# KentaYoshii/Raymarcher

Hardware: AMD Instinct MI355X
Metric: Mpixels/s at 3840x2160 Mandelbulb, 256 march steps (higher is better)
Workload: dtype f32

## Files before the change

raymarcher_amd/csrc/rm_device.hip.h:

```cpp
#pragma once
#include "../../include/raymarcher_amd.h"
#include <type_traits>

#include "rm_math.hip.h"
#include "rm_internal.h"

namespace rm {

struct V3 { float x, y, z; };
struct V4 { float x, y, z, w; };

RM_DEV V3 v3(float x, float y, float z) { return V3{x, y, z}; }
RM_DEV V4 v4(float x, float y, float z, float w) { return V4{x, y, z, w}; }
RM_DEV V3 add(V3 a, V3 b) { return v3(a.x + b.x, a.y + b.y, a.z + b.z); }
RM_DEV V3 sub(V3 a, V3 b) { return v3(a.x - b.x, a.y - b.y, a.z - b.z); }
RM_DEV V3 mul(V3 a, V3 b) { return v3(a.x * b.x, a.y * b.y, a.z * b.z); }
RM_DEV V3 scale(V3 a, float s) { return v3(a.x * s, a.y * s, a.z * s); }
RM_DEV V3 neg(V3 a) { return v3(-a.x, -a.y, -a.z); }
RM_DEV V3 madd(V3 a, float s, V3 b) { return v3(fma(a.x, s, b.x), fma(a.y, s, b.y), fma(a.z, s, b.z)); }
RM_DEV float dot2(float ax, float ay, float bx, float by) { return fma(ay, by, ax * bx); }
RM_DEV float dot(V3 a, V3 b) { return fma(a.z, b.z, fma(a.y, b.y, a.x * b.x)); }
RM_DEV float len2(float x, float y) { return sqrt_(dot2(x, y, x, y)); }
RM_DEV float len(V3 a) { return sqrt_(dot(a, a)); }
RM_DEV V3 normalize(V3 a) { float inv = rcp_(len(a)); return scale(a, inv); }
// ... 472 lines not shown
  const float lipLen = SKIP ? (sb->cullLip * len(rd)) * 1.0001f : 0.0f;
  float ub = ub0;
  float second = -__builtin_inff();
  for (int i = 0; i < steps; i++) {
    const V3 p = madd(rd, depth, ro);
    bool one = false;
    int nearU = 0;
    if (SKIP) {
      nearU = __builtin_amdgcn_readfirstlane(c.idx);
      one = sb->cullOneOk && __ballot(!(c.idx == nearU && nearU >= 0 && second > ub)) == 0ull;
    }
    if (SKIP && one) c = sdSceneOne<COUNT>(sb, nearU, p, cnt);
    else c = sdSceneImpl<BULB, COUNT, !SHADOW, SKIP, SKIP>(sb, p, cnt, ub, second);
    if (fabs_(c.d) < kSurfaceDist || depth > end) break;
    if (SHADOW) {
      if (soft) pen = min_(pen, divr_(8.0f * c.d, depth));
      depth = depth + fabs_(c.d);
    } else {
      depth = fma(c.d, side, depth);
    }
    if (SKIP) {
      ub = nextMinBound(c.d, lipLen, depth);
      second = fma(fabs_(c.d), -(lipLen * 1.0001f), second) - fma(depth, 1.0e-6f, 1.0e-5f);
    }
  }
  MarchRes r;
  bool hit = fabs_(c.d) < kSurfaceDist;
  r.obj = hit ? c.idx : -1;
  r.trap = c.trap;
  if (SHADOW) r.d = pen;
  else r.d = hit ? (depth - c.d) : depth;
  return r;
}

RM_DEV float permute(float x) {
  const float y = fma(x, 34.0f, 1.0f) * x;
  return fma(-289.0f, floor_(RM_DIVC(y, 289.0f)), y);
}
RM_DEV float taylorInvSqrt(float r) { return fma(-0.85373472095314f, r, 1.79284291400159f); }
RM_DEV float fade(float t) { return ((t * t) * t) * fma(t, fma(t, 6.0f, -15.0f), 10.0f); }

RM_DEV void pgrad(float ixyz, float &gx, float &gy, float &gz) {
  float x = RM_DIVC(ixyz, 7.0f);
  float y = fract_(RM_DIVC(floor_(x), 7.0f)) - 0.5f;
  x = fract_(x);
  float z = (0.5f - fabs_(x)) - fabs_(y);
  float sz = step_(z, 0.0f);
  gx = fma(-sz, step_(0.0f, x) - 0.5f, x);
  gy = fma(-sz, step_(0.0f, y) - 0.5f, y);
  gz = z;
}
RM_DEV float pcorner(float ixyz, float fx, float fy, float fz) {
  float gx, gy, gz;
  pgrad(ixyz, gx, gy, gz);
  V3 g = v3(gx, gy, gz);
  g = scale(g, taylorInvSqrt(dot(g, g)));
  return dot(g, v3(fx, fy, fz));
}
RM_DEV float pnoise(V3 p) {
  float i0x = floor_(p.x), i0y = floor_(p.y), i0z = floor_(p.z);
  float i1x = mod_(i0x + 1.0f, 256.0f), i1y = mod_(i0y + 1.0f, 256.0f), i1z = mod_(i0z + 1.0f, 256.0f);
  i0x = mod_(i0x, 256.0f); i0y = mod_(i0y, 256.0f); i0z = mod_(i0z, 256.0f);
  float f0x = fract_(p.x), f0y = fract_(p.y), f0z = fract_(p.z);
  float f1x = f0x - 1.0f, f1y = f0y - 1.0f, f1z = f0z - 1.0f;
  float px0 = permute(i0x), px1 = permute(i1x);
  float ixy00 = permute(px0 + i0y), ixy10 = permute(px1 + i0y);
  float ixy01 = permute(px0 + i1y), ixy11 = permute(px1 + i1y);
  float n000 = pcorner(permute(ixy00 + i0z), f0x, f0y, f0z);
  float n100 = pcorner(permute(ixy10 + i0z), f1x, f0y, f0z);
  float n010 = pcorner(permute(ixy01 + i0z), f0x, f1y, f0z);
  float n110 = pcorner(permute(ixy11 + i0z), f1x, f1y, f0z);
  float n001 = pcorner(permute(ixy00 + i1z), f0x, f0y, f1z);
  float n101 = pcorner(permute(ixy10 + i1z), f1x, f0y, f1z);
  float n011 = pcorner(permute(ixy01 + i1z), f0x, f1y, f1z);
  float n111 = pcorner(permute(ixy11 + i1z), f1x, f1y, f1z);
  float fx = fade(f0x), fy = fade(f0y), fz = fade(f0z);
  float nzx = mix_(n000, n001, fz), nzy = mix_(n100, n101, fz), nzz = mix_(n010, n011, fz), nzw = mix_(n110, n111, fz);
  float nyx = mix_(nzx, nzz, fy), nyy = mix_(nzy, nzw, fy);
  return 2.2f * mix_(nyx, nyy, fx);
}
RM_DEV V3 bumpNormal(V3 normal, V3 pos) {
  V3 ps = scale(pos, 10.0f);
  float nv = pnoise(ps);
  float g[3];
#pragma unroll 1
  for (int k = 0; k < 3; k++) {
    float v = pnoise(v3(ps.x + ((k == 0) ? 0.1f : 0.0f), ps.y + ((k == 1) ? 0.1f : 0.0f),
                        ps.z + ((k == 2) ? 0.1f : 0.0f))) - nv;
    g[0] = (k == 0) ? v : g[0];
    g[1] = (k == 1) ? v : g[1];
    g[2] = (k == 2) ? v : g[2];
  }
  return normalize(madd(v3(g[0], g[1], g[2]), 2.0f, normal));
}

template <int BULB, int COUNT, bool SKIP = false>
RM_DEV float calcAO(const SceneBlock *sb, V3 pos, V3 nor, Counters &cnt, float ubPos = __builtin_inff()) {
  float occ = 0.0f, sca = 1.0f;
  const float lipN = SKIP ? (sb->cullLip * len(nor)) * 1.001f : 0.0f;
  for (int i = 0; i < 5; i++) {
    float h = 0.01f + ((0.12f * (float)i) / 4.0f);
    float d = sdScene<BULB, COUNT, false, SKIP>(sb, madd(nor, h, pos), cnt, SKIP ? fma(h, lipN, ubPos) : ubPos).d;
    occ = fma(h - d, sca, occ);
    sca = sca * 0.95f;
    if (occ > 0.35f) break;
  }
  return clamp_(fma(-3.0f, occ, 1.0f), 0.0f, 1.0f) * fma(0.5f, nor.y, 0.5f);
}
RM_DEV float attenuation(float d, float f0, float f1, float f2) {
  return min_(rcp_(fma(d * d, f2, fma(d, f1, f0))), 1.0f);
}
RM_DEV float angularFalloff(const RmLight &li, V3 L) {
  V3 nd = normalize(v3(li.dir[0], li.dir[1], li.dir[2]));
  float cosalpha = dot(neg(nd), L);
  float inner = li.angle - li.penumbra;
  float t = (acos_(cosalpha) - inner) / (li.angle - inner);
  float mid = 1.0f - fma(-2.0f, pow_(t, 3.0f), 3.0f * pow_(t, 2.0f));
  float r = (cosalpha > cos_(inner)) ? 1.0f : mid;
  return (cosalpha <= cos_(li.angle)) ? 0.0f : r;
}

struct Material { V3 amb, dif, spec; float shininess; };

constexpr float kTextureEps = 0.005f;
constexpr float kGlPi = 3.14159265f;
RM_DEV float uFromTheta(float theta) {
  return (theta < 0.0f) ? (-theta / (2.0f * kGlPi)) : (1.0f - (theta / (2.0f * kGlPi)));
}
RM_DEV void uvMap(int type, V3 p, float rU, float rV, float &su, float &sv) {
  float u, v;
  if (type == RM_CUBE) {
    float ax = fabs_(p.x), ay = fabs_(p.y), az = fabs_(p.z);
    float m = max_(max_(ax, ay), az);
    if (m == ax) { u = (p.x < 0.0f) ? (p.z + 0.5f) : (-p.z + 0.5f); v = p.y + 0.5f; }
    else if (m == ay) { u = p.x + 0.5f; v = (p.y < 0.0f) ? (p.z + 0.5f) : (-p.z + 0.5f); }
    else { u = (p.z < 0.0f) ? (-p.x + 0.5f) : (p.x + 0.5f); v = p.y + 0.5f; }
  } else if (type == RM_SPHERE) {
    u = uFromTheta(atan2_(p.z, p.x));
    float phi = asin_(p.y / 0.5f);
    v = phi / kGlPi + 0.5f;
    if (v == 0.0f || v == 1.0f) u = 0.5f;
  } else {
    bool top = (type == RM_CYLINDER) && (fabs_(p.y - 0.5f) < kTextureEps);
    bool base = fabs_(p.y + 0.5f) < kTextureEps;
    if (top) { u = p.x + 0.5f; v = -p.z + 0.5f; }
    else if (base) { u = p.x + 0.5f; v = p.z + 0.5f; }
    else { u = uFromTheta(atan2_(p.z, p.x)); v = p.y + 0.5f; }
  }
  su = u * rU;
  sv = v * rV;
}
template <bool TEX>
RM_DEV V3 getDiffuse(const SceneBlock *sb, const RmObject &o, V3 p) {
  const float kd = sb->g.kd;
  V3 plain = v3(kd * o.cDiffuse[0], kd * o.cDiffuse[1], kd * o.cDiffuse[2]);
  if (!TEX) return plain;
  if (o.texLoc == -1) return plain;
  const float *M = o.invModel;
  V3 po = v3(fma(M[8], p.z, fma(M[4], p.y, fma(M[0], p.x, M[12]))), fma(M[9], p.z, fma(M[5], p.y, fma(M[1], p.x, M[13]))),
             fma(M[10], p.z, fma(M[6], p.y, fma(M[2], p.x, M[14]))));
  float su, sv;
  uvMap(o.type, po, o.repeatU, o.repeatV, su, sv);
  V3 t = sampleTexture(sb->tex[o.texLoc], su, sv);
  float k = (1.0f - o.blend) * kd;
  return v3(fma(o.blend, t.x, k * o.cDiffuse[0]), fma(o.blend, t.y, k * o.cDiffuse[1]), fma(o.blend, t.z, k * o.cDiffuse[2]));
}

constexpr float kLutScale = (64.0f - 1.0f) / 64.0f, kLutBias = 0.5f / 64.0f;
RM_DEV V3 cross(V3 a, V3 b) {
  return v3(fma(a.y, b.z, -(a.z * b.y)), fma(a.z, b.x, -(a.x * b.z)), fma(a.x, b.y, -(a.y * b.x)));
}
RM_DEV V3 integrateEdgeVec(V3 v1, V3 v2) {
  float x = dot(v1, v2), y = fabs_(x);
  float a = fma(fma(0.0145206f, y, 0.4965155f), y, 0.8543985f);
  float b = fma(4.1616724f + y, y, 3.4175940f);
  float v = a / b;
  float ts = (x > 0.0f) ? v : fma(0.5f, rcp_(sqrt_noscale_(max_(fma(-x, x, 1.0f), 1e-7f))), -v);
  return scale(cross(v1, v2), ts);
}
RM_DEV float ltcEvaluate(const SceneBlock *sb, V3 N, V3 V, V3 P, const M3 &MinvIn, const RmLight &li) {
  V3 T1 = normalize(madd(N, -dot(V, N), V));
  V3 T2 = cross(N, T1);
  M3 B;
  B.c[0][0] = T1.x; B.c[0][1] = T2.x; B.c[0][2] = N.x;
  B.c[1][0] = T1.y; B.c[1][1] = T2.y; B.c[1][2] = N.y;
  B.c[2][0] = T1.z; B.c[2][1] = T2.z; B.c[2][2] = N.z;
  M3 Minv = mulMM(MinvIn, B);
  V3 pts[4], L[4];
#pragma unroll
  for (int k = 0; k < 4; k++) {
    pts[k] = v3(li.points[k][0], li.points[k][1], li.points[k][2]);
    L[k] = normalize(mulMV(Minv, sub(pts[k], P)));
  }
  V3 lightNormal = cross(sub(pts[1], pts[0]), sub(pts[3], pts[0]));
  bool behind = dot(sub(pts[0], P), lightNormal) < 0.0f;
  V3 vsum = integrateEdgeVec(L[0], L[1]);
  vsum = add(vsum, integrateEdgeVec(L[1], L[2]));
  vsum = add(vsum, integrateEdgeVec(L[2], L[3]));
  vsum = add(vsum, integrateEdgeVec(L[3], L[0]));
  float l = len(vsum);
  float z = (l == 0.0f) ? 0.0f : vsum.z / l;
  z = behind ? -z : z;
  float sc = sampleRGBA8<true>(sb->ltc2, RM_LTC_SIZE, RM_LTC_SIZE, fma(fma(z, 0.5f, 0.5f), kLutScale, kLutBias),
                               fma(l, kLutScale, kLutBias)).w;
  float sum = l * sc;
  return (!behind && !li.twoSided) ? 0.0f : sum;
}
RM_DEV V3 getAreaLight(const SceneBlock *sb, V3 N, V3 V, V3 P, const RmLight &li, const Material &mat) {
  float dotNV = clamp_(dot(N, V), 0.0f, 1.0f);
  float u = fma(0.0f, kLutScale, kLutBias), v = fma(sqrt_noscale_(1.0f - dotNV), kLutScale, kLutBias)  ;
  V4 t1 = sampleRGBA8<true>(sb->ltc1, RM_LTC_SIZE, RM_LTC_SIZE, u, v), t2 = sampleRGBA8<true>(sb->ltc2, RM_LTC_SIZE, RM_LTC_SIZE, u, v);
  M3 Minv, I;
#pragma unroll
  for (int c = 0; c < 3; c++)
#pragma unroll
    for (int r = 0; r < 3; r++) { Minv.c[c][r] = (c == 1 && r == 1) ? 1.0f : 0.0f; I.c[c][r] = (c == r) ? 1.0f : 0.0f; }
  Minv.c[0][0] = t1.x; Minv.c[0][2] = t1.y; Minv.c[2][0] = t1.z; Minv.c[2][2] = t1.w;
  float diffuse = ltcEvaluate(sb, N, V, P, I, li);
  float specular = ltcEvaluate(sb, N, V, P, Minv, li);
  float spx = specular * fma(li.intensity - mat.spec.x, t2.y, mat.spec.x * t2.x);
  float spy = specular * fma(li.intensity - mat.spec.y, t2.y, mat.spec.y * t2.x);
  float spz = specular * fma(li.intensity - mat.spec.z, t2.y, mat.spec.z * t2.x);
  return v3((li.color[0] * 1.0f) * fma(mat.dif.x, diffuse, spx), (li.color[1] * 1.0f) * fma(mat.dif.y, diffuse, spy),
            (li.color[2] * 1.0f) * fma(mat.dif.z, diffuse, spz));
}

struct LightGeom { V3 L; float maxT, fAtt, aFall; };
RM_DEV LightGeom lightSetup(const RmLight &li, V3 p, float far) {
  LightGeom g;
  g.fAtt = 1.0f; g.aFall = 1.0f;
  if (li.type == RM_LIGHT_DIRECTIONAL) {
    g.L = normalize(v3(-li.dir[0], -li.dir[1], -li.dir[2]));
    g.maxT = far;
  } else {
    V3 lpos = v3(li.pos[0], li.pos[1], li.pos[2]);
    float d = len(sub(p, lpos));
    V3 toL = sub(lpos, p);
    g.L = normalize(toL);
    g.fAtt = attenuation(d, li.func[0], li.func[1], li.func[2]);
    g.maxT = len(toL);
    if (li.type == RM_LIGHT_SPOT) g.aFall = angularFalloff(li, g.L);
  }
  return g;
}
RM_DEV V3 shadowOrigin(V3 p, V3 N) {
  return v3(fma(N.x * kSurfaceDist, 5.0f, p.x), fma(N.y * kSurfaceDist, 5.0f, p.y), fma(N.z * kSurfaceDist, 5.0f, p.z));
}
RM_DEV bool lightTerm(const RmLight &li, const LightGeom &g, const Material &mat, V3 N, V3 V, float ks,
                      int shadowObj, float pen, bool soft, V3 &cur) {
  float NdotL = dot(N, g.L);
  bool lit = (shadowObj == -1) && !(NdotL <= 0.005f);
  NdotL = clamp_(NdotL, 0.0f, 1.0f);
  V3 lc = v3(li.color[0], li.color[1], li.color[2]);
  cur = v3((mat.dif.x * NdotL) * lc.x, (mat.dif.y * NdotL) * lc.y, (mat.dif.z * NdotL) * lc.z);
  V3 R = reflect(neg(g.L), N);
  float RdotV = clamp_(dot(R, V), 0.0f, 1.0f);
  float sp = (mat.shininess == 0.0f) ? (ks * RdotV) : (ks * pow_(RdotV, mat.shininess));
  cur = v3(fma(sp * mat.spec.x, lc.x, cur.x), fma(sp * mat.spec.y, lc.y, cur.y), fma(sp * mat.spec.z, lc.z, cur.z));
  cur = scale(cur, g.fAtt * g.aFall);
  if (soft) cur = scale(cur, pen);
  return lit;
}

template <int BULB, int COUNT, bool CULLS>
RM_DEV uint32_t shadowQueue(const SceneBlock *sb, V3 so, uint32_t need, float far, Counters &cnt) {
  const int maxSteps = sb->s.maxSteps;
  if (maxSteps <= 0) return 0u;
  uint32_t hitMask = 0u, rest = need;
  int cur = -1, step = 0;
  V3 L = v3(0.0f, 0.0f, 0.0f);
  float depth = 0.0f, end = 0.0f;
  auto nextRay = [&]() {
    cur = rest ? (__builtin_ctz(rest)) : -1;
    rest &= rest - 1u;
    if (cur >= 0) {
      const RmLight &li = sb->lights[cur];
      L = normalize(v3(-li.dir[0], -li.dir[1], -li.dir[2]));
      end = far;
      if (CULLS) end = BULB ? bulbCullEnd(sb, so, L, far) : sceneCullEnd(sb, so, L, far, sb->cullR2);
      depth = 0.0f;
      step = 0;
    }
  };
  nextRay();
  while (__ballot(cur >= 0) != 0ull) {
    if (cur >= 0) {
      const SceneMin c = sdScene<BULB, COUNT, false>(sb, madd(L, depth, so), cnt);
      const bool hit = fabs_(c.d) < kSurfaceDist;
      bool fin = hit || depth > end;
      if (!fin) {
        depth = depth + fabs_(c.d);
        step++;
        fin = step >= maxSteps;
      }
      if (fin) {
        hitMask |= (hit ? 1u : 0u) << cur;
        nextRay();
      }
    }
  }
  return hitMask;
}

template <int BULB, int COUNT, bool RES, bool CULLS, int SPLIT = 0>
RM_DEV V3 getPhong(const SceneBlock *sb, const RmObject *objs, const Material &mat, V3 N, V3 p, V3 rd, float far, Counters &cnt,
                   float ubPos = __builtin_inff(), LightSplit split = LightSplit{-1, nullptr, 0}) {
  constexpr bool SKIP = CULLS && !BULB && COUNT != 1;
  const bool partial = SPLIT == 1 && split.part >= 0;
  const float ka = sb->g.ka, ks = sb->g.ks;
  float ao = 1.0f;
  if (sb->s.enableAmbientOcclusion && !partial) ao = calcAO<BULB, COUNT, SKIP>(sb, p, N, cnt, ubPos);
  const float ubSo = SKIP ? fma(0.005f, (sb->cullLip * len(N)) * 1.001f, ubPos) : ubPos;
  V3 total = v3((mat.amb.x * ka) * ao, (mat.amb.y * ka) * ao, (mat.amb.z * ka) * ao);
  const V3 V = normalize(neg(rd));
  const V3 so = shadowOrigin(p, N);
  const int nl = sb->numLights;
  const bool soft = sb->s.enableSoftShadow != 0;
  if (BULB && !RES && COUNT != 1) {
    bool queue = !soft && nl > 0;
    for (int i = 0; i < nl; i++) queue = queue && sb->lights[i].type == RM_LIGHT_DIRECTIONAL;
    if (queue) {
      uint32_t need = 0u;
      for (int i = 0; i < nl; i++) {
        const RmLight &li = sb->lights[i];
        const V3 L = normalize(v3(-li.dir[0], -li.dir[1], -li.dir[2]));
        if (!(dot(N, L) <= 0.005f)) need |= 1u << i;
      }
      const uint32_t hitMask = shadowQueue<BULB, COUNT, CULLS>(sb, so, need, far, cnt);
      for (int i = 0; i < nl; i++) {
        const RmLight &li = sb->lights[i];
        const LightGeom g = lightSetup(li, p, far);
        V3 cur;
        if (lightTerm(li, g, mat, N, V, ks, ((hitMask >> i) & 1u) ? 0 : -1, 1.0f, false, cur)) total = add(total, cur);
      }
      return total;
    }
  }
  for (int i = 0; i < nl; i++) {
    const RmLight &li = sb->lights[i];
    if (RES && li.type == RM_LIGHT_AREA) {
      V3 p1 = v3(li.points[0][0], li.points[0][1], li.points[0][2]);
      V3 side1 = sub(v3(li.points[1][0], li.points[1][1], li.points[1][2]), p1);
      V3 side2 = sub(v3(li.points[3][0], li.points[3][1], li.points[3][2]), p1);
      V3 toL = sub(madd(side2, rd.y + 0.0f, madd(side1, rd.x + 0.0f, p1)), p);
      V3 L = normalize(toL);
      if (dot(N, L) <= 0.005f) continue;
      MarchRes sh = march<BULB, COUNT, true, CULLS>(sb, so, L, len(toL), 1.0f, cnt, ubSo);
      if (sh.obj != -1 && objs[sh.obj].lightIdx != i) continue;
      total = add(total, getAreaLight(sb, N, V, p, li, mat));
      continue;
    }
    LightGeom g = lightSetup(li, p, far);
    MarchRes sh;
    sh.obj = -1; sh.d = 1.0f; sh.trap = v4(0.0f, 0.0f, 0.0f, 0.0f);
    const bool need = COUNT == 1 || !(dot(N, g.L) <= 0.005f);
    if (partial) {
      if (i == split.part && need) {
        sh = march<BULB, COUNT, true, CULLS>(sb, so, g.L, g.maxT, 1.0f, cnt, ubSo);
        split.slot[2 * i] = __int_as_float(sh.obj);
        split.slot[2 * i + 1] = sh.d;
      }
      continue;
    }
    if (need) {
      if (SPLIT == 2) { sh.obj = __float_as_int(split.slot[2 * i]); sh.d = split.slot[2 * i + 1]; }
      else sh = march<BULB, COUNT, true, CULLS>(sb, so, g.L, g.maxT, 1.0f, cnt, ubSo);
    }
    V3 cur;
    if (lightTerm(li, g, mat, N, V, ks, sh.obj, sh.d, soft, cur)) total = add(total, cur);
  }
  return total;
}

RM_DEV V3 bulbTrapColor(float ty, float tz, float tw) {
  V3 c = v3(0.2f, 0.2f, 0.2f);
  c = mix(c, v3(0.10f, 0.20f, 0.30f), clamp_(ty, 0.0f, 1.0f));
  c = mix(c, v3(0.02f, 0.10f, 0.30f), clamp_(tz * tz, 0.0f, 1.0f));
  c = mix(c, v3(0.30f, 0.10f, 0.02f), clamp_(pow_(tw, 6.0f), 0.0f, 1.0f));
  return scale(c, 0.5f);
}

template <int BULB, int COUNT, bool TEX, bool CULLS, int SPLIT = 0>
RM_DEV RenderOut render(const SceneBlock *sb, const RmObject *objs, V3 ro, V3 rd, Hit &info, float side, float maxT,
                        V3 bg, Counters &cnt, LightSplit split = LightSplit{-1, nullptr, 0}) {
  RenderOut out;
  info.obj = -1;
  MarchRes res;
  if (SPLIT == 2) {
    const float *q = split.slot + 2 * sb->numLights;
    res.obj = __float_as_int(q[0]); res.d = q[1]; res.trap = v4(q[2], q[3], q[4], q[5]);
  } else {
    res = march<BULB, COUNT, false, CULLS>(sb, ro, rd, maxT, side, cnt);
    if (SPLIT == 1 && split.part == 0) {
      float *q = split.slot + 2 * sb->numLights;
      q[0] = __int_as_float(res.obj); q[1] = res.d; q[2] = res.trap.x; q[3] = res.trap.y; q[4] = res.trap.z; q[5] = res.trap.w;
    }
  }
  if (res.obj == -1) {
    out.col = (TEX && sb->s.enableSkyBox) ? sampleCube(sb->skybox, rd) : bg;
    out.isEnv = 1;
    out.d = maxT;
    return out;
  }
  out.isEnv = 0;
  out.d = res.d;
  if (COUNT) cnt.shades++;
  V3 p = madd(rd, res.d, ro);
  constexpr bool SKIP = CULLS && !BULB && COUNT != 1;
  float ubP = __builtin_inff();
  if (SKIP) {
    const float lipLen = (sb->cullLip * len(rd)) * 1.0001f;
    ubP = fma(kSurfaceDist, lipLen, kSurfaceDist) * 1.001f + fma(fabs_(res.d), 1.0e-6f, 1.0e-5f);
  }
  V3 pn = getNormal<BULB, COUNT, SKIP>(sb, p, cnt, SKIP ? fma(0.0005f, sb->cullLip * 1.001f, ubP) : ubP);
  if (sb->s.features & RM_FEAT_PERLIN_BUMP) pn = bumpNormal(pn, p);
  const RmObject &o = objs[BULB ? 0 : res.obj];
  if (TEX && o.isEmissive) {
    out.col = v3(o.color[0], o.color[1], o.color[2]);
    return out;
  }
  Material mat;
  mat.amb = v3(o.cAmbient[0], o.cAmbient[1], o.cAmbient[2]);
  mat.dif = getDiffuse<TEX>(sb, o, p);
  mat.spec = v3(o.cSpecular[0], o.cSpecular[1], o.cSpecular[2]);
  mat.shininess = o.shininess;
  const int type = BULB ? (int)RM_MANDELBULB : o.type;
  V3 ph = getPhong<BULB, COUNT, TEX, CULLS, SPLIT>(sb, objs, mat, pn, p, rd, maxT, cnt, ubP, split);
  V3 col = ph;
  if (type == RM_MANDELBULB) {
    V3 c = bulbTrapColor(res.trap.y, res.trap.z, res.trap.w);
    col = v3(c.x * (ph.x * 8.0f), c.y * (ph.y * 8.0f), c.z * (ph.z * 8.0f));
  } else if (type == RM_MENGERSPONGE) {
    V3 c = v3(fma(0.5f, cos_(fma(2.0f, res.trap.z, 0.0f)), 0.5f), fma(0.5f, cos_(fma(2.0f, res.trap.z, 1.0f)), 0.5f),
              fma(0.5f, cos_(fma(2.0f, res.trap.z, 2.0f)), 0.5f));
    col = mul(c, ph);
  }
  info.p = p; info.n = pn; info.rd = rd; info.obj = res.obj;
  out.col = col;
  return out;
}

struct QuadCoord { float I, J; bool upper; };
RM_DEV QuadCoord quadCoord(int px, int py, int W, int H) {
  const float tx = ((float)px + 0.5f) / (float)W, ty = ((float)py + 0.5f) / (float)H;
  QuadCoord q;
  q.upper = (tx + ty) > 1.0f;
  q.I = q.upper ? 1.0f - tx : tx;
  q.J = q.upper ? 1.0f - ty : ty;
  return q;
}
RM_DEV void pixelNdc(int px, int py, int W, int H, float &ndcx, float &ndcy) {
  const QuadCoord q = quadCoord(px, py, W, H);
  ndcx = q.upper ? fma(q.I, -2.0f, 1.0f) : fma(q.I, 2.0f, -1.0f);
  ndcy = q.upper ? fma(q.J, -2.0f, 1.0f) : fma(q.J, 2.0f, -1.0f);
}
RM_DEV void primaryRay(const SceneBlock *sb, int px, int py, int W, int H, V3 &ro, V3 &rd) {
  const QuadCoord q = quadCoord(px, py, W, H);
  float nc[4], fc4[4];
#pragma unroll
  for (int k = 0; k < 4; k++) {
    const float (*A)[3][4] = sb->rayPlane[0], (*B)[3][4] = sb->rayPlane[1];
    auto sc = [](float v) { return u2f((uint32_t)__builtin_amdgcn_readfirstlane((int)f2u(v))); };
    const float p0n = q.upper ? sc(B[0][0][k]) : sc(A[0][0][k]), p1n = q.upper ? sc(B[0][1][k]) : sc(A[0][1][k]),
                p2n = q.upper ? sc(B[0][2][k]) : sc(A[0][2][k]);
    const float p0f = q.upper ? sc(B[1][0][k]) : sc(A[1][0][k]), p1f = q.upper ? sc(B[1][1][k]) : sc(A[1][1][k]),
                p2f = q.upper ? sc(B[1][2][k]) : sc(A[1][2][k]);
    nc[k] = fma(q.J, p2n, fma(q.I, p1n, p0n));
    fc4[k] = fma(q.J, p2f, fma(q.I, p1f, p0f));
  }
  ro = v3(nc[0] / nc[3], nc[1] / nc[3], nc[2] / nc[3]);
  V3 fc = v3(fc4[0] / fc4[3], fc4[1] / fc4[3], fc4[2] / fc4[3]);
  rd = normalize(sub(fc, ro));
}
RM_DEV V3 backgroundColor(const SceneBlock *sb) {
  V3 bg = v3(0.0f, 0.0f, 0.0f);
  if (sb->s.features & RM_FEAT_WHITE_BACKGROUND) bg = v3(1.0f, 1.0f, 1.0f);
  if (sb->s.features & RM_FEAT_DARK_BACKGROUND) bg = v3(0.0f, 0.0f, 0.0f);
  return bg;
}
RM_DEV V3 backgroundColor(const SceneBlock *sb, V3 rd) {
  V3 bg = v3(0.0f, 0.0f, 0.0f);
  if (sb->s.features & RM_FEAT_SKY_BACKGROUND) bg = getSky(rd);
  if (sb->s.features & RM_FEAT_NIGHTSKY_BACKGROUND) bg = getMoonColor(sb->noise, sb->g.iTime, rd);
  if (sb->s.features & RM_FEAT_WHITE_BACKGROUND) bg = v3(1.0f, 1.0f, 1.0f);
  if (sb->s.features & RM_FEAT_DARK_BACKGROUND) bg = v3(0.0f, 0.0f, 0.0f);
  return bg;
}

template <int BULB, int COUNT, bool ENV, bool TEX, bool SEC = true, int SPLIT = 0, bool BATCH = false>
RM_DEV void shadePixel(const SceneBlock *sb, const RmObject *objs, int px, int py, int W, int H, V4 &fragColor,
                       V4 &bright, Counters &cnt, bool &hitFlag, LightSplit split = LightSplit{-1, nullptr, 0}) {
  float ndcx, ndcy;
  pixelNdc(px, py, W, H, ndcx, ndcy);
  bright = v4(0.0f, 0.0f, 0.0f, 1.0f);
  hitFlag = false;
  if (sb->g.isTwoD) {
    float s = sdMandelBrot(sb, ndcx, ndcy);
    fragColor = v4(pow_(s, 0.9f), pow_(s, 1.1f), pow_(s, 1.4f), 1.0f);
    return;
  }
  V3 ro, rd;
  primaryRay(sb, px, py, W, H, ro, rd);
  const V3 bg = ENV ? backgroundColor(sb, rd) : backgroundColor(sb);
  const uint32_t feat = sb->s.features;
  const bool env = ENV && (feat & (RM_FEAT_TERRAIN | RM_FEAT_CLOUD | RM_FEAT_SEA)) != 0;
  const float far = (ENV && (feat & RM_FEAT_CLOUD)) ? 2000.0f : sb->cam.initialFar;
  const float iTime = sb->g.iTime;

  Hit info;
  RenderOut ri = render<BULB, COUNT, TEX, !ENV, SPLIT>(sb, objs, ro, rd, info, 1.0f, far, bg, cnt, split);
  EnvOut e;
  e.terrainHit = false; e.cloudHit = false; e.seaHit = false;
  if (env) e = envLayers(feat, sb->noise, iTime, W, ro, rd, ri.d, bg, cnt);
  if (ri.isEnv && !e.cloudHit && !e.terrainHit && !e.seaHit) {
    fragColor = v4(ri.col.x, ri.col.y, ri.col.z, 1.0f);
    return;
  }
  if (e.cloudHit || e.terrainHit || e.seaHit) {
    V3 c = e.cloudHit ? e.ccol : (e.terrainHit ? e.tcol : e.scol);
    fragColor = v4(c.x, c.y, c.z, 1.0f);
    if (dot(c, v3(0.2126f, 0.7152f, 0.0722f)) > 1.0f) bright = v4(c.x, c.y, c.z, 1.0f);
    return;
  }
  hitFlag = true;
  V4 phong = v4(ri.col.x, ri.col.y, ri.col.z, 1.0f);
  V4 refl = v4(0.0f, 0.0f, 0.0f, 0.0f), refr = v4(0.0f, 0.0f, 0.0f, 0.0f);
  const Hit oi = info;
  const bool noObj = TEX && info.obj < 0;
  const RmObject &o = objs[(BULB || noObj) ? 0 : info.obj];
  const V3 cRefl = noObj ? v3(0.0f, 0.0f, 0.0f) : v3(o.cReflective[0], o.cReflective[1], o.cReflective[2]);
  const V3 cRefr = noObj ? v3(0.0f, 0.0f, 0.0f) : v3(o.cTransparent[0], o.cTransparent[1], o.cTransparent[2]);
  const float ior = o.ior;
  if (SEC && sb->s.enableReflection && len(cRefl) != 0.0f) {
    V3 fil = v3(1.0f, 1.0f, 1.0f);
    const int nb = sb->s.numReflection;
    for (int i = 0; i < nb; i++) {
      V3 r = reflect(info.rd, info.n);
      V3 sro = v3(fma(r.x * kSurfaceDist, 3.0f, info.p.x), fma(r.y * kSurfaceDist, 3.0f, info.p.y),
                  fma(r.z * kSurfaceDist, 3.0f, info.p.z));
      fil = mul(fil, cRefl);
      RenderOut res = render<BULB, COUNT, TEX, !ENV>(sb, objs, sro, r, info, 1.0f, far, bg, cnt);
      if (env) {
        EnvOut b = envLayers(feat, sb->noise, iTime, W, sro, r, res.d, bg, cnt);
        if (b.seaHit) res.col = b.scol;
        if (b.terrainHit) { res.col = b.tcol; res.isEnv = 1; }
        if (b.cloudHit) { res.col = b.ccol; res.isEnv = 1; }
      }
      refl.x += (sb->g.ks * fil.x) * res.col.x;
      refl.y += (sb->g.ks * fil.y) * res.col.y;
      refl.z += (sb->g.ks * fil.z) * res.col.z;
      refl.w += 1.0f;
      if (res.isEnv) break;
    }
  }
  if (SEC && sb->s.enableRefraction && len(cRefr) != 0.0f) {
    V3 rdIn = refract(oi.rd, oi.n, 1.0f / ior);
    V3 pEnter = v3(fma(-(oi.n.x * kSurfaceDist), 3.0f, oi.p.x), fma(-(oi.n.y * kSurfaceDist), 3.0f, oi.p.y),
                   fma(-(oi.n.z * kSurfaceDist), 3.0f, oi.p.z));
    float dIn = march<BULB, COUNT, false>(sb, pEnter, rdIn, far, -1.0f, cnt).d;
    V3 pExit = madd(rdIn, dIn, pEnter);
    V3 nExit = neg(getNormal<BULB, COUNT>(sb, pExit, cnt));
    V3 rdOut = refract(rdIn, nExit, ior);
    if (len(rdOut) != 0.0f) {
      V3 sro = v3(fma(-(nExit.x * kSurfaceDist), 5.0f, pExit.x), fma(-(nExit.y * kSurfaceDist), 5.0f, pExit.y),
                  fma(-(nExit.z * kSurfaceDist), 5.0f, pExit.z));
      RenderOut res = render<BULB, COUNT, TEX, !ENV>(sb, objs, sro, rdOut, info, 1.0f, far, bg, cnt);
      if (env) {
        EnvOut b = envLayers(feat, sb->noise, iTime, W, sro, rdOut, res.d, bg, cnt);
        if (b.seaHit) res.col = b.scol;
        if (b.terrainHit) res.col = b.tcol;
        if (b.cloudHit) res.col = b.ccol;
      }
      refr.x += (sb->g.kt * cRefr.x) * res.col.x;
      refr.y += (sb->g.kt * cRefr.y) * res.col.y;
      refr.z += (sb->g.kt * cRefr.z) * res.col.z;
      refr.w += 1.0f;
    }
  }
  fragColor = v4((phong.x + refl.x) + refr.x, (phong.y + refl.y) + refr.y, (phong.z + refl.z) + refr.z,
                 (phong.w + refl.w) + refr.w);
  V3 c = v3(fragColor.x, fragColor.y, fragColor.z);
  float brightness = dot(c, v3(0.2126f, 0.7152f, 0.0722f));
  if (brightness > 1.0f) bright = v4(c.x, c.y, c.z, 1.0f);
}

}
```

Measured before the change: 4372.

## Pool shadow rays across wavefront lanes for Mandelbulb hard directional lights

Adds a wave-level shadow ray pool. Each lane pushes its pending (pixel, light) shadow rays into an LDS list, and idle lanes (including lanes whose primary ray missed) pick up work from it until the list drains. Hits are written back through per-wave atomic bitmasks. It also evaluates the first shadow SDF step per pixel once and reuses it as the starting depth for every light. The aim is to cut SIMD divergence in the shadow march, at the cost of LDS use, ballots and shuffles, and an assumption of 256-thread blocks (4 waves of 64).

Measured after the change: 4565 (median of 6 runs). +4.4%, better.

```diff
diff --git a/raymarcher_amd/csrc/rm_device.hip.h b/raymarcher_amd/csrc/rm_device.hip.h
--- a/raymarcher_amd/csrc/rm_device.hip.h
+++ b/raymarcher_amd/csrc/rm_device.hip.h
@@ -798,6 +798,24 @@
   return hitMask;
 }
 
+RM_DEV bool hardDirectionalOnly(const SceneBlock *sb) {
+  const int nl = sb->numLights;
+  bool ok = sb->s.enableSoftShadow == 0 && nl > 0;
+  for (int i = 0; i < nl; i++) ok = ok && sb->lights[i].type == RM_LIGHT_DIRECTIONAL;
+  return ok;
+}
+RM_DEV V3 hardLightSum(const SceneBlock *sb, const Material &mat, V3 N, V3 p, V3 V, float far, float ks, uint32_t hitMask,
+                       V3 total) {
+  const int nl = sb->numLights;
+  for (int i = 0; i < nl; i++) {
+    const RmLight &li = sb->lights[i];
+    const LightGeom g = lightSetup(li, p, far);
+    V3 cur;
+    if (lightTerm(li, g, mat, N, V, ks, ((hitMask >> i) & 1u) ? 0 : -1, 1.0f, false, cur)) total = add(total, cur);
+  }
+  return total;
+}
+
 template <int BULB, int COUNT, bool RES, bool CULLS, int SPLIT = 0>
 RM_DEV V3 getPhong(const SceneBlock *sb, const RmObject *objs, const Material &mat, V3 N, V3 p, V3 rd, float far, Counters &cnt,
                    float ubPos = __builtin_inff(), LightSplit split = LightSplit{-1, nullptr, 0}) {
@@ -813,9 +831,7 @@
   const int nl = sb->numLights;
   const bool soft = sb->s.enableSoftShadow != 0;
   if (BULB && !RES && COUNT != 1) {
-    bool queue = !soft && nl > 0;
-    for (int i = 0; i < nl; i++) queue = queue && sb->lights[i].type == RM_LIGHT_DIRECTIONAL;
-    if (queue) {
+    if (hardDirectionalOnly(sb)) {
       uint32_t need = 0u;
       for (int i = 0; i < nl; i++) {
         const RmLight &li = sb->lights[i];
@@ -823,13 +839,7 @@
         if (!(dot(N, L) <= 0.005f)) need |= 1u << i;
       }
       const uint32_t hitMask = shadowQueue<BULB, COUNT, CULLS>(sb, so, need, far, cnt);
-      for (int i = 0; i < nl; i++) {
-        const RmLight &li = sb->lights[i];
-        const LightGeom g = lightSetup(li, p, far);
-        V3 cur;
-        if (lightTerm(li, g, mat, N, V, ks, ((hitMask >> i) & 1u) ? 0 : -1, 1.0f, false, cur)) total = add(total, cur);
-      }
-      return total;
+      return hardLightSum(sb, mat, N, p, V, far, ks, hitMask, total);
     }
   }
   for (int i = 0; i < nl; i++) {
@@ -876,7 +886,135 @@
   return scale(c, 0.5f);
 }
 
-template <int BULB, int COUNT, bool TEX, bool CULLS, int SPLIT = 0>
+constexpr int kPoolWaves = 4, kPoolList = 64 * RM_MAX_LIGHTS;
+static_assert(RM_MAX_LIGHTS <= 16, "a pool entry holds the light in 10 bits, a hit mask 16 lights");
+template <int BULB, int COUNT>
+RM_DEV uint32_t shadowPool(const SceneBlock *sb, V3 so, uint32_t pend, float dStart, float far, Counters &cnt) {
+  __shared__ uint16_t s_list[kPoolWaves][kPoolList];
+  __shared__ uint32_t s_hits[kPoolWaves][32];
+  const int wave = (int)(threadIdx.x >> 6), lane = (int)__lane_id();
+  uint16_t *list = s_list[wave];
+  uint32_t *hitw = s_hits[wave];
+  hitw[lane >> 1] = 0u;
+  const int nl = sb->numLights;
+  uint32_t n = 0u;
+  for (int i = 0; i < nl; i++) {
+    const bool mine = ((pend >> i) & 1u) != 0u;
+    const uint64_t m = __ballot(mine);
+    const uint32_t rank = __builtin_amdgcn_mbcnt_hi((uint32_t)(m >> 32), __builtin_amdgcn_mbcnt_lo((uint32_t)m, 0u));
+    if (mine) list[n + rank] = (uint16_t)(lane | (i << 6));
+    n += (uint32_t)__popcll(m);
+  }
+  __builtin_amdgcn_wave_barrier();
+  const int maxSteps = sb->s.maxSteps;
+  int cur = -1, own = 0, step = 0;
+  V3 o = so, L = v3(0.0f, 0.0f, 0.0f);
+  float depth = 0.0f, end = 0.0f;
+  uint32_t next = 0u;
+  for (;;) {
+    const uint64_t idle = __ballot(cur < 0);
+    if (idle != 0ull && next < n) {
+      const uint32_t k = next + __builtin_amdgcn_mbcnt_hi((uint32_t)(idle >> 32), __builtin_amdgcn_mbcnt_lo((uint32_t)idle, 0u));
+      next += (uint32_t)__popcll(idle);
+      const bool take = cur < 0 && k < n;
+      uint32_t e = 0u;
+      if (take) e = list[k];
+      const int src = (int)(e & 63u);
+      const V3 os = v3(__shfl(so.x, src), __shfl(so.y, src), __shfl(so.z, src));
+      const float ds = __shfl(dStart, src);
+      if (take) {
+        cur = (int)(e >> 6);
+        own = src;
+        o = os;
+        const RmLight &li = sb->lights[cur];
+        L = normalize(v3(-li.dir[0], -li.dir[1], -li.dir[2]));
+        end = bulbCullEnd(sb, o, L, far);
+        const bool resume = !(ds < 0.0f);
+        depth = resume ? ds : 0.0f;
+        step = resume ? 1 : 0;
+        if (resume && 0.0f > end) cur = -1;
+      }
+    }
+    if (cur >= 0) {
+      const SceneMin c = sdScene<BULB, COUNT, false>(sb, madd(L, depth, o), cnt);
+      const bool hit = fabs_(c.d) < kSurfaceDist;
+      bool fin = hit || depth > end;
+      if (!fin) {
+        depth = depth + fabs_(c.d);
+        step++;
+        fin = step >= maxSteps;
+      }
+      if (fin) {
+        if (hit) atomicOr(&hitw[own >> 1], 1u << (((own & 1) << 4) + cur));
+        cur = -1;
+      }
+    }
+    if (__ballot(cur >= 0) == 0ull && next >= n) break;
+  }
+  __builtin_amdgcn_wave_barrier();
+  return (hitw[lane >> 1] >> ((lane & 1) << 4)) & 0xffffu;
+}
+
+template <int BULB, int COUNT>
+RM_DEV RenderOut renderPooled(const SceneBlock *sb, const RmObject *objs, V3 ro, V3 rd, const MarchRes &res, Hit &info,
+                              float maxT, V3 bg, Counters &cnt) {
+  const bool surf = res.obj != -1;
+  const int nl = sb->numLights;
+  V3 p = v3(0.0f, 0.0f, 0.0f), N = p, so = p;
+  float ao = 1.0f, dStart = -1.0f;
+  uint32_t pend = 0u, hits = 0u;
+  if (surf) {
+    if (COUNT) cnt.shades++;
+    p = madd(rd, res.d, ro);
+    N = getNormal<BULB, COUNT>(sb, p, cnt);
+    if (sb->s.features & RM_FEAT_PERLIN_BUMP) N = bumpNormal(N, p);
+    if (sb->s.enableAmbientOcclusion) ao = calcAO<BULB, COUNT>(sb, p, N, cnt);
+    so = shadowOrigin(p, N);
+    bool shared = f2u(so.x) != 0x80000000u && f2u(so.y) != 0x80000000u && f2u(so.z) != 0x80000000u;
+    uint32_t need = 0u;
+    for (int i = 0; i < nl; i++) {
+      const RmLight &li = sb->lights[i];
+      const V3 L = normalize(v3(-li.dir[0], -li.dir[1], -li.dir[2]));
+      shared = shared && (fabs_(L.x) + fabs_(L.y) + fabs_(L.z) <= 2.0f);
+      if (!(dot(N, L) <= 0.005f)) need |= 1u << i;
+    }
+    const int maxSteps = sb->s.maxSteps;
+    if (need != 0u && maxSteps > 0) {
+      if (!shared) {
+        pend = need;
+      } else {
+        const float d0 = fabs_(sdScene<BULB, COUNT, false>(sb, so, cnt).d);
+        if (d0 < kSurfaceDist) hits = need;
+        else if (maxSteps > 1) { pend = need; dStart = d0; }
+      }
+    }
+  }
+  const uint32_t hitMask = hits | shadowPool<BULB, COUNT>(sb, so, pend, dStart, maxT, cnt);
+  RenderOut out;
+  if (!surf) {
+    out.col = bg;
+    out.isEnv = 1;
+    out.d = maxT;
+    return out;
+  }
+  out.isEnv = 0;
+  out.d = res.d;
+  const RmObject &o = objs[0];
+  Material mat;
+  mat.amb = v3(o.cAmbient[0], o.cAmbient[1], o.cAmbient[2]);
+  mat.dif = getDiffuse<false>(sb, o, p);
+  mat.spec = v3(o.cSpecular[0], o.cSpecular[1], o.cSpecular[2]);
+  mat.shininess = o.shininess;
+  const float ka = sb->g.ka, ks = sb->g.ks;
+  const V3 total = v3((mat.amb.x * ka) * ao, (mat.amb.y * ka) * ao, (mat.amb.z * ka) * ao);
+  const V3 ph = hardLightSum(sb, mat, N, v3(0.0f, 0.0f, 0.0f), normalize(neg(rd)), maxT, ks, hitMask, total);
+  const V3 c = bulbTrapColor(res.trap.y, res.trap.z, res.trap.w);
+  out.col = v3(c.x * (ph.x * 8.0f), c.y * (ph.y * 8.0f), c.z * (ph.z * 8.0f));
+  info.p = p; info.n = N; info.rd = rd; info.obj = res.obj;
+  return out;
+}
+
+template <int BULB, int COUNT, bool TEX, bool CULLS, int SPLIT = 0, bool POOL = false>
 RM_DEV RenderOut render(const SceneBlock *sb, const RmObject *objs, V3 ro, V3 rd, Hit &info, float side, float maxT,
                         V3 bg, Counters &cnt, LightSplit split = LightSplit{-1, nullptr, 0}) {
   RenderOut out;
@@ -892,6 +1030,7 @@
       q[0] = __int_as_float(res.obj); q[1] = res.d; q[2] = res.trap.x; q[3] = res.trap.y; q[4] = res.trap.z; q[5] = res.trap.w;
     }
   }
+  if (POOL && hardDirectionalOnly(sb)) return renderPooled<BULB, COUNT>(sb, objs, ro, rd, res, info, maxT, bg, cnt);
   if (res.obj == -1) {
     out.col = (TEX && sb->s.enableSkyBox) ? sampleCube(sb->skybox, rd) : bg;
     out.isEnv = 1;
@@ -1004,7 +1143,8 @@
   const float iTime = sb->g.iTime;
 
   Hit info;
-  RenderOut ri = render<BULB, COUNT, TEX, !ENV, SPLIT>(sb, objs, ro, rd, info, 1.0f, far, bg, cnt, split);
+  constexpr bool POOL = BULB && !ENV && !TEX && COUNT != 1 && SPLIT == 0;
+  RenderOut ri = render<BULB, COUNT, TEX, !ENV, SPLIT, POOL>(sb, objs, ro, rd, info, 1.0f, far, bg, cnt, split);
   EnvOut e;
   e.terrainHit = false; e.cloudHit = false; e.seaHit = false;
   if (env) e = envLayers(feat, sb->noise, iTime, W, ro, rd, ri.d, bg, cnt);
```
